# LightwheelAI/street-gaussians-ns

Measured on NVIDIA H100. Metric: rendered frames/sec (fwd+bwd) at 1920x1280, 1M+32x10k Gaussians, higher is better.
Workload: dtype f32

## Files before the change

street-gaussians-ns_b200/csrc/project.cu:

```cuda
#include <stdarg.h>
#include <stdlib.h>
#include <string.h>

#include "sgn_exact.cuh"
#include "sgn_touch.cuh"

static thread_local char g_err[512] = "";
void sgn_set_error(const char* fmt, ...) {
    va_list ap;
    va_start(ap, fmt);
    vsnprintf(g_err, sizeof(g_err), fmt, ap);
    va_end(ap);
}
#include <atomic>
static std::atomic<long long> g_launches{0};
void sgn_count_launch(int n) { g_launches.fetch_add(n, std::memory_order_relaxed); }
extern "C" long long sgn_launch_count(void) { return g_launches.load(std::memory_order_relaxed); }
extern "C" const char* sgn_last_error(void) { return g_err; }
extern "C" int sgn_abi_version(void) { return SGN_ABI_VERSION; }
extern "C" size_t sgn_sizeof_segment(void) { return sizeof(sgn_segment); }
extern "C" size_t sgn_sizeof_segment_grads(void) { return sizeof(sgn_segment_grads); }
extern "C" size_t sgn_sizeof_camera(void) { return sizeof(sgn_camera); }

extern "C" int sgn_upload(const void* host, size_t bytes, void* dev, void* stream) {
    SGN_RANGE("sgn_upload");
    SGN_REQUIRE(host && dev, "sgn_upload: null pointer");
    SGN_CHECK_CUDA(cudaMemcpyAsync(dev, host, bytes, cudaMemcpyHostToDevice, (cudaStream_t)stream));
    return SGN_OK;
}

#define SGN_MAX_SEGMENTS 1024
#define PROJ_THREADS 256
#define CH 128
#define MAX_REST 45
#define MAX_DC (3 * SGN_MAX_FOURIER)

__device__ __forceinline__ sgn_camera sgn_camera_with_view(const sgn_camera& c, const float* __restrict__ view) {
    sgn_camera o = c;
#pragma unroll
    for (int k = 0; k < 12; ++k) o.viewmat[k] = __ldg(view + k);
#pragma unroll
    for (int k = 0; k < 3; ++k) o.cam_pos[k] = __ldg(view + 12 + k);
    return o;
}

__device__ __forceinline__ int find_segment_by_chunk(const int* s_chunk0, int nseg, int c) {
    int lo = 0, hi = nseg - 1;
    while (lo < hi) {
        const int mid = (lo + hi + 1) >> 1;
        if (s_chunk0[mid] <= c) lo = mid; else hi = mid - 1;
    }
    return lo;
}

__device__ __forceinline__ void coop_load(float* __restrict__ dst, const float* __restrict__ src, int n) {
    if ((reinterpret_cast<uintptr_t>(src) & 15u) == 0) {
        const int n4 = n >> 2;
        const float4* s4 = reinterpret_cast<const float4*>(src);
        float4* d4 = reinterpret_cast<float4*>(dst);
        for (int i = threadIdx.x; i < n4; i += blockDim.x) d4[i] = __ldg(s4 + i);
        for (int i = (n4 << 2) + threadIdx.x; i < n; i += blockDim.x) dst[i] = __ldg(src + i);
    } else {
        for (int i = threadIdx.x; i < n; i += blockDim.x) dst[i] = __ldg(src + i);
    }
}
__device__ __forceinline__ void coop_store(float* __restrict__ dst, const float* __restrict__ src, int n) {
    if ((reinterpret_cast<uintptr_t>(dst) & 15u) == 0) {
        const int n4 = n >> 2;
        const float4* s4 = reinterpret_cast<const float4*>(src);
        float4* d4 = reinterpret_cast<float4*>(dst);
        for (int i = threadIdx.x; i < n4; i += blockDim.x) d4[i] = s4[i];
        for (int i = (n4 << 2) + threadIdx.x; i < n; i += blockDim.x) dst[i] = src[i];
    } else {
        for (int i = threadIdx.x; i < n; i += blockDim.x) dst[i] = src[i];
    }
}

template <bool VIEW>
__global__ void __launch_bounds__(CH)
project_fwd_direct_kernel(const sgn_segment* __restrict__ segs, int nseg, const sgn_camera cam_arg,
                   float4* __restrict__ records, int32_t* __restrict__ radii, int32_t* __restrict__ num_tiles_hit,
                   ushort4* __restrict__ tile_bbox, int32_t* __restrict__ tiles_touched, uint32_t* __restrict__ touch_mask,
                   const float* __restrict__ view) {
    sgn_camera cam_view;
    if constexpr (VIEW) cam_view = sgn_camera_with_view(cam_arg, view);
    const sgn_camera& cam = VIEW ? cam_view : cam_arg;
    extern __shared__ int s_chunk0[];
    for (int i = threadIdx.x; i < nseg; i += blockDim.x) s_chunk0[i] = segs[i].chunk0;
    __syncthreads();
    const int si = find_segment_by_chunk(s_chunk0, nseg, blockIdx.x);
    const sgn_segment& sg = segs[si];
    const int i = (blockIdx.x - sg.chunk0) * CH + threadIdx.x;
    const bool active = i < sg.count;
    const size_t g = (size_t)sg.row0 + i;
    const int K = (cam.sh_degree + 1) * (cam.sh_degree + 1);
    bool vis = false;
    ushort4 bb = make_ushort4(0, 0, 0, 0);
    TouchCtx tc = {};
    if (active) {

    float m[3], ls[3], q[4];
#pragma unroll
    for (int k = 0; k < 3; ++k) { m[k] = __ldg(sg.means + 3 * (size_t)i + k); ls[k] = __ldg(sg.scales + 3 * (size_t)i + k); }
    {
        const float4 qq = __ldg(reinterpret_cast<const float4*>(sg.quats) + i);
        q[0] = qq.x; q[1] = qq.y; q[2] = qq.z; q[3] = qq.w;
    }
    const bool filt = cam.filter_3d != nullptr;
    const float sigma = filt ? __ldg(cam.filter_3d[si] + i) : 0.f;
    SgnProj st;
    vis = sgn_project_exact(sg, cam, m, ls, q, st, true, 1.f, cam.antialiased != 0, filt, sigma);

    float rgb[3] = {0.f, 0.f, 0.f};
    float opac = 0.f, comp = 0.f;
    int aux = 0;
    if (vis) {
        float c0[3] = {0.f, 0.f, 0.f};
        for (int f = 0; f < sg.F; ++f) {
            const float w = sg.idft[f];
#pragma unroll
            for (int ch = 0; ch < 3; ++ch) c0[ch] += __ldg(sg.features_dc + ((size_t)i * sg.F + f) * 3 + ch) * w;
        }
        if (cam.sh_degree > 0) {
            float d[3] = {st.mw[0] - cam.cam_pos[0], st.mw[1] - cam.cam_pos[1], st.mw[2] - cam.cam_pos[2]};
            const float n = sqrtf(d[0] * d[0] + d[1] * d[1] + d[2] * d[2]);
            d[0] /= n; d[1] /= n; d[2] /= n;
            float Y[16];
            sgn_sh_basis(cam.sh_degree_to_use, d[0], d[1], d[2], Y);
            const int Kuse = min((cam.sh_degree_to_use + 1) * (cam.sh_degree_to_use + 1), K);
            float acc[3] = {Y[0] * c0[0], Y[0] * c0[1], Y[0] * c0[2]};
            const float* rest = sg.features_rest + (size_t)i * (K - 1) * 3;
            for (int k = 1; k < Kuse; ++k) {
#pragma unroll
                for (int ch = 0; ch < 3; ++ch) acc[ch] += Y[k] * __ldg(rest + (k - 1) * 3 + ch);
            }
#pragma unroll
            for (int ch = 0; ch < 3; ++ch) {
                const float pre = acc[ch] + 0.5f;
                if (pre >= 0.f) aux |= (1 << ch);
                rgb[ch] = pre > 0.f ? pre : 0.f;
            }
        } else {
#pragma unroll
            for (int ch = 0; ch < 3; ++ch) { rgb[ch] = 1.f / (1.f + expf(-c0[ch])); aux |= (1 << ch); }
        }
        opac = 1.f / (1.f + expf(-__ldg(sg.opacities + i)));
        if (filt) opac = opac * st.coef;
        if (cam.antialiased) {
            comp = st.comp;
            opac = opac * comp;
        }
        aux |= SGN_AUX_VISIBLE;
    }
    if (sg.cls == 1) aux |= SGN_AUX_OBJECT;

    float4* rec = records + 3 * g;
    rec[0] = make_float4(st.xy[0], st.xy[1], st.conic[0], st.conic[1]);
    rec[1] = make_float4(st.conic[2], opac, rgb[0], rgb[1]);
    rec[2] = make_float4(rgb[2], vis ? st.pv[2] : 0.f, __int_as_float(aux), comp);
    radii[g] = st.radius;
    num_tiles_hit[g] = vis ? (st.tmax[0] - st.tmin[0]) * (st.tmax[1] - st.tmin[1]) : 0;
    bb = make_ushort4((unsigned short)st.tmin[0], (unsigned short)st.tmin[1],
                      (unsigned short)st.tmax[0], (unsigned short)st.tmax[1]);
    tile_bbox[g] = bb;
    if (vis) tc = make_touch_ctx(make_float4(st.xy[0], st.xy[1], st.conic[0], st.conic[1]), make_float4(st.conic[2], opac, 0.f, 0.f));
    }
    uint32_t mask;
    const int nt = count_touched_tiles(vis, tc, bb, cam.width, cam.height, cam.block_width, mask);
    if (active) {
        tiles_touched[g] = nt;
        touch_mask[g] = mask;
    }
}

__global__ void __launch_bounds__(CH)
project_fwd_staged_kernel(const sgn_segment* __restrict__ segs, int nseg, const sgn_camera cam,
                   float4* __restrict__ records, int32_t* __restrict__ radii, int32_t* __restrict__ num_tiles_hit,
                   ushort4* __restrict__ tile_bbox, int32_t* __restrict__ tiles_touched, uint32_t* __restrict__ touch_mask) {
    extern __shared__ int s_chunk0[];
    __shared__ __align__(16) float s_rest[CH * MAX_REST];
    __shared__ __align__(16) float s_dc[CH * MAX_DC];
    __shared__ __align__(16) float s_means[CH * 3];
    __shared__ __align__(16) float s_scales[CH * 3];
    __shared__ float s_geo[CH][11];
    __shared__ int s_row[CH];
    __shared__ int s_warp_base[CH / 32 + 1];
    for (int i = threadIdx.x; i < nseg; i += blockDim.x) s_chunk0[i] = segs[i].chunk0;
    __syncthreads();
    const int si = find_segment_by_chunk(s_chunk0, nseg, blockIdx.x);
    const sgn_segment& sg = segs[si];
    const int r0 = (blockIdx.x - sg.chunk0) * CH;
    const int rows = min(CH, sg.count - r0);
    const int tid = threadIdx.x, lane = tid & 31, warp = tid >> 5;
    const int K = (cam.sh_degree + 1) * (cam.sh_degree + 1);
    const int nrest = (K - 1) * 3, ndc = sg.F * 3;
    coop_load(s_means, sg.means + 3 * (size_t)r0, rows * 3);
    coop_load(s_scales, sg.scales + 3 * (size_t)r0, rows * 3);
    __syncthreads();

    const bool active = tid < rows;
    const size_t g = (size_t)sg.row0 + r0 + tid;
    const int cls_bit = sg.cls == 1 ? SGN_AUX_OBJECT : 0;
    bool vis = false;
    SgnProj st;
    if (active) {
        const float m[3] = {s_means[3 * tid], s_means[3 * tid + 1], s_means[3 * tid + 2]};
        const float ls[3] = {s_scales[3 * tid], s_scales[3 * tid + 1], s_scales[3 * tid + 2]};
        const float4 qq = __ldg(reinterpret_cast<const float4*>(sg.quats) + r0 + tid);
        const float q[4] = {qq.x, qq.y, qq.z, qq.w};
        const bool filt = cam.filter_3d != nullptr;
        const float sigma = filt ? __ldg(cam.filter_3d[si] + r0 + tid) : 0.f;
        vis = sgn_project_exact(sg, cam, m, ls, q, st, true, 1.f, cam.antialiased != 0, filt, sigma);
        radii[g] = st.radius;
        num_tiles_hit[g] = vis ? (st.tmax[0] - st.tmin[0]) * (st.tmax[1] - st.tmin[1]) : 0;
        tile_bbox[g] = make_ushort4((unsigned short)st.tmin[0], (unsigned short)st.tmin[1],
                                    (unsigned short)st.tmax[0], (unsigned short)st.tmax[1]);
        float4* rec = records + 3 * g;
        rec[0] = make_float4(st.xy[0], st.xy[1], st.conic[0], st.conic[1]);
        if (!vis) {
            rec[1] = make_float4(st.conic[2], 0.f, 0.f, 0.f);
            rec[2] = make_float4(0.f, 0.f, __int_as_float(cls_bit), 0.f);
            tiles_touched[g] = 0;
            touch_mask[g] = 0u;
        }
    }
    const unsigned bal = __ballot_sync(0xffffffffu, vis);
    if (lane == 0) s_warp_base[warp + 1] = __popc(bal);
    __syncthreads();
    if (tid == 0) {
        s_warp_base[0] = 0;
#pragma unroll
        for (int w = 0; w < CH / 32; ++w) s_warp_base[w + 1] += s_warp_base[w];
    }
    __syncthreads();
    const int nvis = s_warp_base[CH / 32];
    if (vis) {
        const int c = s_warp_base[warp] + __popc(bal & ((1u << lane) - 1u));
        s_row[c] = tid;
        float* ge = s_geo[c];
        ge[0] = st.xy[0]; ge[1] = st.xy[1]; ge[2] = st.conic[0]; ge[3] = st.conic[1]; ge[4] = st.conic[2];
        ge[5] = st.pv[2]; ge[6] = st.mw[0]; ge[7] = st.mw[1]; ge[8] = st.mw[2];
        ge[9] = st.comp;
        ge[10] = st.coef;
    }
    __syncthreads();
    if (nvis == 0) return;

    {
        const unsigned inv_rest = nrest > 0 ? (0xffffffffu / (unsigned)nrest) + 1u : 0u;
        const float* __restrict__ rest = sg.features_rest + (size_t)r0 * nrest;
        const int n_rest = nvis * nrest;
        for (int e0 = tid; e0 < n_rest; e0 += 4 * CH) {
            float v[4];
#pragma unroll
            for (int u = 0; u < 4; ++u) {
                const int e = e0 + u * CH;
                if (e < n_rest) {
                    const int r = (int)__umulhi((unsigned)e, inv_rest);
                    v[u] = __ldg(rest + s_row[r] * nrest + (e - r * nrest));
                }
            }
#pragma unroll
            for (int u = 0; u < 4; ++u) {
                const int e = e0 + u * CH;
                if (e < n_rest) s_rest[e] = v[u];
            }
        }
        const unsigned inv_dc = (0xffffffffu / (unsigned)ndc) + 1u;
        const float* __restrict__ dc = sg.features_dc + (size_t)r0 * ndc;
        for (int e = tid; e < nvis * ndc; e += CH) {
            const int r = (int)__umulhi((unsigned)e, inv_dc);
            s_dc[e] = __ldg(dc + s_row[r] * ndc + (e - r * ndc));
        }
    }
    __syncthreads();

    const bool mine = tid < nvis;
    ushort4 bb = make_ushort4(0, 0, 0, 0);
    TouchCtx tc = {};
    size_t gb = 0;
    if (mine) {
        const int row = s_row[tid];
        gb = (size_t)sg.row0 + r0 + row;
        const float* ge = s_geo[tid];
        float c0[3] = {0.f, 0.f, 0.f};
        const float* dcr = s_dc + tid * ndc;
        for (int f = 0; f < sg.F; ++f) {
            const float w = sg.idft[f];
#pragma unroll
            for (int ch = 0; ch < 3; ++ch) c0[ch] += dcr[f * 3 + ch] * w;
        }
        float rgb[3];
        int aux = SGN_AUX_VISIBLE | cls_bit;
        if (cam.sh_degree > 0) {
            float d[3] = {ge[6] - cam.cam_pos[0], ge[7] - cam.cam_pos[1], ge[8] - cam.cam_pos[2]};
            const float n = sqrtf(d[0] * d[0] + d[1] * d[1] + d[2] * d[2]);
            d[0] /= n; d[1] /= n; d[2] /= n;
            float Y[16];
            sgn_sh_basis(cam.sh_degree_to_use, d[0], d[1], d[2], Y);
            const int Kuse = min((cam.sh_degree_to_use + 1) * (cam.sh_degree_to_use + 1), K);
            float acc[3] = {Y[0] * c0[0], Y[0] * c0[1], Y[0] * c0[2]};
            const float* rr = s_rest + tid * nrest;
            for (int k = 1; k < Kuse; ++k) {
#pragma unroll
                for (int ch = 0; ch < 3; ++ch) acc[ch] += Y[k] * rr[(k - 1) * 3 + ch];
            }
#pragma unroll
            for (int ch = 0; ch < 3; ++ch) {
                const float pre = acc[ch] + 0.5f;
                if (pre >= 0.f) aux |= (1 << ch);
                rgb[ch] = pre > 0.f ? pre : 0.f;
            }
        } else {
#pragma unroll
            for (int ch = 0; ch < 3; ++ch) { rgb[ch] = 1.f / (1.f + expf(-c0[ch])); aux |= (1 << ch); }
        }
        float opac = 1.f / (1.f + expf(-__ldg(sg.opacities + r0 + row)));
        if (cam.filter_3d) opac = opac * ge[10];
        if (cam.antialiased) opac = opac * ge[9];
        float4* rec = records + 3 * gb;
        rec[1] = make_float4(ge[4], opac, rgb[0], rgb[1]);
        rec[2] = make_float4(rgb[2], ge[5], __int_as_float(aux), ge[9]);
        bb = tile_bbox[gb];
        tc = make_touch_ctx(make_float4(ge[0], ge[1], ge[2], ge[3]), make_float4(ge[4], opac, 0.f, 0.f));
    }
    if ((warp << 5) >= nvis) return;
    uint32_t mask;
    const int nt = count_touched_tiles(mine, tc, bb, cam.width, cam.height, cam.block_width, mask);
    if (mine) {
        tiles_touched[gb] = nt;
        touch_mask[gb] = mask;
    }
}

static int project_fwd_check(const char* what, const sgn_segment* segs_dev, int nseg, int N, int num_chunks, const sgn_camera* cam,
                             float* records, int32_t* radii, int32_t* num_tiles_hit, uint16_t* tile_bbox,
                             int32_t* tiles_touched, uint32_t* touch_mask) {
    SGN_REQUIRE(segs_dev && cam && records && radii && num_tiles_hit && tile_bbox && tiles_touched && touch_mask,
                "%s: null pointer", what);
    SGN_REQUIRE(nseg >= 1 && nseg <= SGN_MAX_SEGMENTS, "%s: nseg=%d out of range [1,%d]", what, nseg, SGN_MAX_SEGMENTS);
    SGN_REQUIRE(N >= 0 && num_chunks >= 0, "%s: negative size", what);
    SGN_REQUIRE(cam->block_width >= 2 && cam->block_width <= 16, "block_width must be between 2 and 16 (got %d)", cam->block_width);
    SGN_REQUIRE(cam->sh_degree >= 0 && cam->sh_degree <= 3 && cam->sh_degree_to_use >= 0 && cam->sh_degree_to_use <= cam->sh_degree,
                "sh_degree must be in [0,3] and sh_degree_to_use <= sh_degree");
    SGN_REQUIRE((cam->width + cam->block_width - 1) / cam->block_width < 65536 && (cam->height + cam->block_width - 1) / cam->block_width < 65536,
                "image too large for 16-bit tile coordinates");
    SGN_REQUIRE(sgn_aligned16(records), "records must be 16-byte aligned");
    return SGN_OK;
}

extern "C" int sgn_project_fwd_view(const sgn_segment* segs_dev, int nseg, int N, int num_chunks, const sgn_camera* cam,
                                    const float* view, float* records, int32_t* radii, int32_t* num_tiles_hit, uint16_t* tile_bbox,
                                    int32_t* tiles_touched, uint32_t* touch_mask, void* stream) {
    SGN_RANGE("sgn_project_fwd_view");
    if (int rc = project_fwd_check("sgn_project_fwd_view", segs_dev, nseg, N, num_chunks, cam, records, radii, num_tiles_hit, tile_bbox,
                                   tiles_touched, touch_mask)) return rc;
    SGN_REQUIRE(view, "sgn_project_fwd_view: null view");
    if (N == 0 || num_chunks == 0) return SGN_OK;
    project_fwd_direct_kernel<true><<<num_chunks, CH, nseg * sizeof(int), (cudaStream_t)stream>>>(
        segs_dev, nseg, *cam, reinterpret_cast<float4*>(records), radii, num_tiles_hit,
        reinterpret_cast<ushort4*>(tile_bbox), tiles_touched, touch_mask, view);
    SGN_CHECK_LAUNCH("project_fwd_kernel<view>");
    return SGN_OK;
}

extern "C" int sgn_project_fwd(const sgn_segment* segs_dev, int nseg, int N, int num_chunks, const sgn_camera* cam,
                               float* records, int32_t* radii, int32_t* num_tiles_hit, uint16_t* tile_bbox,
                               int32_t* tiles_touched, uint32_t* touch_mask, void* stream) {
    SGN_RANGE("sgn_project_fwd");
    if (int rc = project_fwd_check("sgn_project_fwd", segs_dev, nseg, N, num_chunks, cam, records, radii, num_tiles_hit, tile_bbox,
                                   tiles_touched, touch_mask)) return rc;
    if (N == 0 || num_chunks == 0) return SGN_OK;
    const char* staged_env = getenv("SGN_PROJECT_STAGED");
    if (staged_env && staged_env[0] == '1')
        project_fwd_staged_kernel<<<num_chunks, CH, nseg * sizeof(int), (cudaStream_t)stream>>>(
            segs_dev, nseg, *cam, reinterpret_cast<float4*>(records), radii, num_tiles_hit,
            reinterpret_cast<ushort4*>(tile_bbox), tiles_touched, touch_mask);
    else
        project_fwd_direct_kernel<false><<<num_chunks, CH, nseg * sizeof(int), (cudaStream_t)stream>>>(
            segs_dev, nseg, *cam, reinterpret_cast<float4*>(records), radii, num_tiles_hit,
            reinterpret_cast<ushort4*>(tile_bbox), tiles_touched, touch_mask, nullptr);
    SGN_CHECK_LAUNCH("project_fwd_kernel");
    return SGN_OK;
}

template <bool VIEW = false>
__device__ __forceinline__ void sgn_project_vjp(const sgn_camera& cam, const SgnProj& st, const float v_xy[2], float v_depth,
                                                const float v_conic[3], float vmw[3], float vs[3], float vqr[4],
                                                float* vview = nullptr, bool with_comp = false, float comp = 0.f,
                                                float v_comp = 0.f) {
    const float* W = cam.viewmat;
    const float fx = cam.fx, fy = cam.fy;
    float vpv[3];
    {
        const float rw = 1.f / (st.pv[2] + 1e-6f);
        const float vx = fx * v_xy[0], vy = fy * v_xy[1];
        vpv[0] = vx * rw;
        vpv[1] = vy * rw;
        vpv[2] = -(vx * st.pv[0] + vy * st.pv[1]) * rw * rw + v_depth;
    }
    float vA, vB, vC;
    {
        const float X0 = st.conic[0], X1 = st.conic[1], X2 = st.conic[2];
        const float G0 = v_conic[0], G1 = 0.5f * v_conic[1], G2 = v_conic[2];
        const float a00 = X0 * G0 + X1 * G1, a01 = X0 * G1 + X1 * G2;
        const float a10 = X1 * G0 + X2 * G1, a11 = X1 * G1 + X2 * G2;
        vA = -(a00 * X0 + a01 * X1);
        vB = -(a00 * X1 + a01 * X2) - (a10 * X0 + a11 * X1);
        vC = -(a10 * X1 + a11 * X2);
    }
    if (with_comp) {
        xf T[6], S[6], a, b, c, c00, c11;
#pragma unroll
        for (int k = 0; k < 6; ++k) { T[k] = xf(st.T[k]); S[k] = xf(st.S[k]); }
        sgn_cov2d_blur(T, S, a, b, c, c00, c11);
        sgn_compensation_vjp(c00.v, c11.v, a.v, b.v, c.v, comp, v_comp, vA, vB, vC);
    }
    const float g00 = vA, g01 = 0.5f * vB, g11 = vC;
    const float* T = st.T;
    const float Sf[9] = {st.S[0], st.S[1], st.S[2], st.S[1], st.S[3], st.S[4], st.S[2], st.S[4], st.S[5]};
    float GT[6];
#pragma unroll
    for (int c = 0; c < 3; ++c) {
        GT[c] = g00 * T[c] + g01 * T[3 + c];
        GT[3 + c] = g01 * T[c] + g11 * T[3 + c];
    }
    float vS[9];
#pragma unroll
    for (int r = 0; r < 3; ++r)
#pragma unroll
        for (int c = 0; c < 3; ++c) vS[3 * r + c] = T[r] * GT[c] + T[3 + r] * GT[3 + c];
    float vT[6];
#pragma unroll
    for (int r = 0; r < 2; ++r)
#pragma unroll
        for (int c = 0; c < 3; ++c)
            vT[3 * r + c] = 2.f * (GT[3 * r] * Sf[c] + GT[3 * r + 1] * Sf[3 + c] + GT[3 * r + 2] * Sf[6 + c]);
    const float vJ00 = vT[0] * W[0] + vT[1] * W[1] + vT[2] * W[2];
    const float vJ02 = vT[0] * W[8] + vT[1] * W[9] + vT[2] * W[10];
    const float vJ11 = vT[3] * W[4] + vT[4] * W[5] + vT[5] * W[6];
    const float vJ12 = vT[3] * W[8] + vT[4] * W[9] + vT[5] * W[10];
    {
        const float rz = 1.f / st.pv[2], rz2 = rz * rz, rz3 = rz2 * rz;
        const float vtx = -fx * rz2 * vJ02;
        const float vty = -fy * rz2 * vJ12;
        const float vtz = -fx * rz2 * vJ00 - fy * rz2 * vJ11 + 2.f * fx * st.tx * rz3 * vJ02 + 2.f * fy * st.ty * rz3 * vJ12;
        if (st.clampx == 0) vpv[0] += vtx; else vpv[2] += (st.clampx > 0 ? cam.limx : -cam.limx) * vtx;
        if (st.clampy == 0) vpv[1] += vty; else vpv[2] += (st.clampy > 0 ? cam.limy : -cam.limy) * vty;
        vpv[2] += vtz;
        if constexpr (VIEW) {
            const float J00 = fx * rz, J11 = fy * rz, J02 = -fx * st.tx * rz2, J12 = -fy * st.ty * rz2;
#pragma unroll
            for (int c = 0; c < 3; ++c) {
                vview[c] = vpv[0] * st.mw[c] + J00 * vT[c];
                vview[4 + c] = vpv[1] * st.mw[c] + J11 * vT[3 + c];
                vview[8 + c] = vpv[2] * st.mw[c] + J02 * vT[c] + J12 * vT[3 + c];
            }
#pragma unroll
            for (int r = 0; r < 3; ++r) vview[4 * r + 3] = vpv[r];
        }
    }
#pragma unroll
    for (int c = 0; c < 3; ++c) vmw[c] = W[c] * vpv[0] + W[4 + c] * vpv[1] + W[8 + c] * vpv[2];
    float M[9], vM[9];
#pragma unroll
    for (int r = 0; r < 3; ++r)
#pragma unroll
        for (int c = 0; c < 3; ++c) M[3 * r + c] = st.Rg[3 * r + c] * st.s[c];
#pragma unroll
    for (int r = 0; r < 3; ++r)
#pragma unroll
        for (int c = 0; c < 3; ++c)
            vM[3 * r + c] = 2.f * (vS[3 * r] * M[c] + vS[3 * r + 1] * M[3 + c] + vS[3 * r + 2] * M[6 + c]);
    float vR[9];
#pragma unroll
    for (int c = 0; c < 3; ++c) {
        vs[c] = st.Rg[c] * vM[c] + st.Rg[3 + c] * vM[3 + c] + st.Rg[6 + c] * vM[6 + c];
#pragma unroll
        for (int r = 0; r < 3; ++r) vR[3 * r + c] = vM[3 * r + c] * st.s[c];
    }
    float vqn[4];
    {
        const float w = st.qn[0], x = st.qn[1], y = st.qn[2], z = st.qn[3];
        vqn[0] = 2.f * (x * (vR[7] - vR[5]) + y * (vR[2] - vR[6]) + z * (vR[3] - vR[1]));
        vqn[1] = 2.f * (-2.f * x * (vR[4] + vR[8]) + y * (vR[1] + vR[3]) + z * (vR[2] + vR[6]) + w * (vR[7] - vR[5]));
        vqn[2] = 2.f * (x * (vR[1] + vR[3]) - 2.f * y * (vR[0] + vR[8]) + z * (vR[5] + vR[7]) + w * (vR[2] - vR[6]));
        vqn[3] = 2.f * (x * (vR[2] + vR[6]) + y * (vR[5] + vR[7]) - 2.f * z * (vR[0] + vR[4]) + w * (vR[3] - vR[1]));
    }
    const float dot = vqn[0] * st.qn[0] + vqn[1] * st.qn[1] + vqn[2] * st.qn[2] + vqn[3] * st.qn[3];
#pragma unroll
    for (int k = 0; k < 4; ++k) vqr[k] = (vqn[k] - st.qn[k] * dot) / st.qnorm;
}

template <bool POSE, bool VIEW = false>
__global__ void __launch_bounds__(CH)
project_bwd_kernel(const sgn_segment* __restrict__ segs, const sgn_segment_grads* __restrict__ grads, int nseg,
                   const sgn_camera cam_arg, const float4* __restrict__ records, const int32_t* __restrict__ radii,
                   const float4* __restrict__ v_records, const int chunk_begin, float* __restrict__ pose_partials,
                   const float* __restrict__ view, float* __restrict__ view_partials) {
    sgn_camera cam_view;
    if constexpr (VIEW) cam_view = sgn_camera_with_view(cam_arg, view);
    const sgn_camera& cam = VIEW ? cam_view : cam_arg;
    extern __shared__ int s_chunk0[];
    __shared__ __align__(16) float s_rest[CH * MAX_REST];
    __shared__ __align__(16) float s_dc[CH * MAX_DC];
    __shared__ __align__(16) float s_means[CH * 3];
    __shared__ __align__(16) float s_scales[CH * 3];
    for (int i = threadIdx.x; i < nseg; i += blockDim.x) s_chunk0[i] = segs[i].chunk0;
    __syncthreads();
    const int chunk = chunk_begin + (int)blockIdx.x;
    const int si = find_segment_by_chunk(s_chunk0, nseg, chunk);
    const sgn_segment& sg = segs[si];
    const sgn_segment_grads& gr = grads[si];
    const int r0 = (chunk - sg.chunk0) * CH;
    const int rows = min(CH, sg.count - r0);
    const int K = (cam.sh_degree + 1) * (cam.sh_degree + 1);
    const int nrest = (K - 1) * 3, ndc = sg.F * 3;
    coop_load(s_means, sg.means + 3 * (size_t)r0, rows * 3);
    coop_load(s_scales, sg.scales + 3 * (size_t)r0, rows * 3);
    __syncthreads();
    const int tid = threadIdx.x;
    float gm[3] = {0.f, 0.f, 0.f}, gs[3] = {0.f, 0.f, 0.f}, gq[4] = {0.f, 0.f, 0.f, 0.f};
    float vp[POSE ? SGN_POSE_FLOATS : 1] = {};
    float vv[VIEW ? SGN_VIEW_FLOATS : 1] = {};
    const bool row_vis = (tid < rows) && radii[(size_t)sg.row0 + r0 + tid] > 0;
    if (tid < rows && !row_vis) {
        const int i = r0 + tid;
        gr.opacities[i] = 0.f;
        reinterpret_cast<float4*>(gr.quats)[i] = make_float4(0.f, 0.f, 0.f, 0.f);
        float* grest = s_rest + tid * nrest;
        for (int k = 0; k < nrest; ++k) grest[k] = 0.f;
        float* gdc = s_dc + tid * ndc;
        for (int k = 0; k < ndc; ++k) gdc[k] = 0.f;
    }
    if (row_vis) {
        const int i = r0 + tid;
        const size_t g = (size_t)sg.row0 + i;
        const float4 v0 = v_records[3 * g], v1 = v_records[3 * g + 1], v2 = v_records[3 * g + 2];
        const float v_xy[2] = {v0.x, v0.y};
        const float v_conic[3] = {v0.z, v0.w, v1.x};
        const float v_opac = v1.y;
        const float v_rgb[3] = {v1.z, v1.w, v2.x};
        const float v_depth = v2.y;
        const float4 r1 = records[3 * g + 1], r2 = records[3 * g + 2];
        const int aux = __float_as_int(r2.z);
        const bool filt = cam.filter_3d != nullptr;
        if (!cam.antialiased && !filt) {
            const float o = r1.y;
            gr.opacities[i] = v_opac * o * (1.f - o);
        }
        const float m[3] = {s_means[3 * tid], s_means[3 * tid + 1], s_means[3 * tid + 2]};
        const float ls[3] = {s_scales[3 * tid], s_scales[3 * tid + 1], s_scales[3 * tid + 2]};
        float q[4];
        {
            const float4 qq = __ldg(reinterpret_cast<const float4*>(sg.quats) + i);
            q[0] = qq.x; q[1] = qq.y; q[2] = qq.z; q[3] = qq.w;
        }
        const float sigma = filt ? __ldg(cam.filter_3d[si] + i) : 0.f;
        SgnProj st;
        const bool vis = sgn_project_exact(sg, cam, m, ls, q, st, true, 1.f, false, filt, sigma);
        {
            float vc[3];
            float* grest = s_rest + tid * nrest;
            if (cam.sh_degree > 0) {
                float d[3] = {st.mw[0] - cam.cam_pos[0], st.mw[1] - cam.cam_pos[1], st.mw[2] - cam.cam_pos[2]};
                const float n = sqrtf(d[0] * d[0] + d[1] * d[1] + d[2] * d[2]);
                d[0] /= n; d[1] /= n; d[2] /= n;
                float Y[16];
                sgn_sh_basis(cam.sh_degree_to_use, d[0], d[1], d[2], Y);
                const int Kuse = (cam.sh_degree_to_use + 1) * (cam.sh_degree_to_use + 1);
#pragma unroll
                for (int ch = 0; ch < 3; ++ch) vc[ch] = (aux & (1 << ch)) ? v_rgb[ch] : 0.f;
                for (int k = 1; k < K; ++k) {
                    const float y = (k < Kuse) ? Y[k] : 0.f;
#pragma unroll
                    for (int ch = 0; ch < 3; ++ch) grest[(k - 1) * 3 + ch] = y * vc[ch];
                }
#pragma unroll
                for (int ch = 0; ch < 3; ++ch) vc[ch] *= Y[0];
            } else {
                const float rgb[3] = {r1.z, r1.w, r2.x};
#pragma unroll
                for (int ch = 0; ch < 3; ++ch) vc[ch] = v_rgb[ch] * rgb[ch] * (1.f - rgb[ch]);
                for (int k = 0; k < nrest; ++k) grest[k] = 0.f;
            }
            float* gdc = s_dc + tid * ndc;
            for (int f = 0; f < sg.F; ++f) {
                const float w = sg.idft[f];
#pragma unroll
                for (int ch = 0; ch < 3; ++ch) gdc[f * 3 + ch] = w * vc[ch];
            }
        }
        float v_comp = 0.f, comp = 0.f, v_coef = 0.f;
        if (cam.antialiased || filt) {
            const float s = 1.f / (1.f + expf(-__ldg(sg.opacities + i)));
            float f = 1.f;
            if (cam.antialiased) {
                v_comp = v_opac * s;
                f = r2.w;
                comp = __ldg(reinterpret_cast<const float*>(records) + 12 * g + 11);
            }
            if (filt) {
                v_coef = v_opac * s * f;
                v_comp = v_comp * st.coef;
                f = f * st.coef;
            }
            gr.opacities[i] = v_opac * f * s * (1.f - s);
        }
        if (vis && radii[g] > 0) {
            float vmw[3], vs[3], vqr[4];
            sgn_project_vjp<VIEW>(cam, st, v_xy, v_depth, v_conic, vmw, vs, vqr, vv, cam.antialiased != 0, comp, v_comp);
#pragma unroll
            for (int c = 0; c < 3; ++c) gs[c] = vs[c] * st.s[c];
            if (filt) {
                float r[3];
                sgn_filter_ratios(ls, sigma, r);
                const float vc = v_coef * st.coef;
#pragma unroll
                for (int c = 0; c < 3; ++c) gs[c] = gs[c] * r[c] + vc * (1.f - r[c]);
            }
            if (sg.has_pose) {
                const float* R = sg.R;
#pragma unroll
                for (int c = 0; c < 3; ++c) gm[c] = R[c] * vmw[0] + R[3 + c] * vmw[1] + R[6 + c] * vmw[2];
                const float aw = sg.q[0], ax = sg.q[1], ay = sg.q[2], az = sg.q[3];
                gq[0] = aw * vqr[0] + ax * vqr[1] + ay * vqr[2] + az * vqr[3];
                gq[1] = -ax * vqr[0] + aw * vqr[1] + az * vqr[2] - ay * vqr[3];
                gq[2] = -ay * vqr[0] - az * vqr[1] + aw * vqr[2] + ax * vqr[3];
                gq[3] = -az * vqr[0] + ay * vqr[1] - ax * vqr[2] + aw * vqr[3];
                if constexpr (POSE) {
#pragma unroll
                    for (int r = 0; r < 3; ++r) {
#pragma unroll
                        for (int c = 0; c < 3; ++c) vp[3 * r + c] = vmw[r] * m[c];
                        vp[9 + r] = vmw[r];
                    }
                    vp[12] = vqr[0] * q[0] + vqr[1] * q[1] + vqr[2] * q[2] + vqr[3] * q[3];
                    vp[13] = -vqr[0] * q[1] + vqr[1] * q[0] - vqr[2] * q[3] + vqr[3] * q[2];
                    vp[14] = -vqr[0] * q[2] + vqr[1] * q[3] + vqr[2] * q[0] - vqr[3] * q[1];
                    vp[15] = -vqr[0] * q[3] - vqr[1] * q[2] + vqr[2] * q[1] + vqr[3] * q[0];
                }
            } else {
#pragma unroll
                for (int c = 0; c < 3; ++c) gm[c] = vmw[c];
#pragma unroll
                for (int k = 0; k < 4; ++k) gq[k] = vqr[k];
            }
        }
        reinterpret_cast<float4*>(gr.quats)[i] = make_float4(gq[0], gq[1], gq[2], gq[3]);
    }
    if constexpr (POSE) {
        __shared__ float s_pose[(CH / 32) * SGN_POSE_FLOATS];
        if (sg.has_pose) {
#pragma unroll
            for (int k = 0; k < SGN_POSE_FLOATS; ++k) {
                float x = vp[k];
#pragma unroll
                for (int o = 16; o > 0; o >>= 1) x += __shfl_down_sync(0xffffffffu, x, o);
                if ((tid & 31) == 0) s_pose[(tid >> 5) * SGN_POSE_FLOATS + k] = x;
            }
            __syncthreads();
            if (tid < SGN_POSE_FLOATS) {
                float x = s_pose[tid];
#pragma unroll
                for (int w = 1; w < CH / 32; ++w) x += s_pose[w * SGN_POSE_FLOATS + tid];
                pose_partials[(size_t)chunk * SGN_POSE_FLOATS + tid] = x;
            }
        }
    }
    if constexpr (VIEW) {
        __shared__ float s_view[(CH / 32) * SGN_VIEW_FLOATS];
#pragma unroll
        for (int k = 0; k < SGN_VIEW_FLOATS; ++k) {
            float x = vv[k];
#pragma unroll
            for (int o = 16; o > 0; o >>= 1) x += __shfl_down_sync(0xffffffffu, x, o);
            if ((tid & 31) == 0) s_view[(tid >> 5) * SGN_VIEW_FLOATS + k] = x;
        }
        __syncthreads();
        if (tid < SGN_VIEW_FLOATS) {
            float x = s_view[tid];
#pragma unroll
            for (int w = 1; w < CH / 32; ++w) x += s_view[w * SGN_VIEW_FLOATS + tid];
            view_partials[(size_t)chunk * SGN_VIEW_FLOATS + tid] = x;
        }
    }
// ... 255 lines not shown
```

Before: 438.3.

## Stage SH rest features via per-warp cp.async and coalesce record stores through smem

The projection forward kernel now gathers the SH rest coefficients of visible Gaussians into per-warp shared memory with cp.async. This overlaps the gather with the opacity, DC colour and tile-bbox work, replacing strided per-thread global loads. The 48-byte per-Gaussian records are first written to shared memory and then stored to global memory in a coalesced warp loop. The env-selected staged kernel is removed. The kernel now carries a large static shared-memory buffer, which may lower occupancy.

```diff
diff --git a/street-gaussians-ns_b200/csrc/project.cu b/street-gaussians-ns_b200/csrc/project.cu
--- a/street-gaussians-ns_b200/csrc/project.cu
+++ b/street-gaussians-ns_b200/csrc/project.cu
@@ -76,9 +76,17 @@
     }
 }
 
+__device__ __forceinline__ uint32_t smem_u32(const void* p) { return (uint32_t)__cvta_generic_to_shared(p); }
+__device__ __forceinline__ void cp_async4(void* dst, const void* src) {
+    asm volatile("cp.async.ca.shared.global [%0], [%1], 4;\n" ::"r"(smem_u32(dst)), "l"(src) : "memory");
+}
+__device__ __forceinline__ void cp_async_commit() { asm volatile("cp.async.commit_group;\n" ::: "memory"); }
+template <int N>
+__device__ __forceinline__ void cp_async_wait() { asm volatile("cp.async.wait_group %0;\n" ::"n"(N) : "memory"); }
+
 template <bool VIEW>
 __global__ void __launch_bounds__(CH)
-project_fwd_direct_kernel(const sgn_segment* __restrict__ segs, int nseg, const sgn_camera cam_arg,
+project_fwd_kernel(const sgn_segment* __restrict__ segs, int nseg, const sgn_camera cam_arg,
                    float4* __restrict__ records, int32_t* __restrict__ radii, int32_t* __restrict__ num_tiles_hit,
                    ushort4* __restrict__ tile_bbox, int32_t* __restrict__ tiles_touched, uint32_t* __restrict__ touch_mask,
                    const float* __restrict__ view) {
@@ -86,53 +94,85 @@
     if constexpr (VIEW) cam_view = sgn_camera_with_view(cam_arg, view);
     const sgn_camera& cam = VIEW ? cam_view : cam_arg;
     extern __shared__ int s_chunk0[];
+    __shared__ __align__(16) float s_rest[CH / 32][32 * MAX_REST];
+    __shared__ int s_vrow[CH];
     for (int i = threadIdx.x; i < nseg; i += blockDim.x) s_chunk0[i] = segs[i].chunk0;
     __syncthreads();
     const int si = find_segment_by_chunk(s_chunk0, nseg, blockIdx.x);
     const sgn_segment& sg = segs[si];
-    const int i = (blockIdx.x - sg.chunk0) * CH + threadIdx.x;
+    const int lane = threadIdx.x & 31, warp = threadIdx.x >> 5;
+    const int r0 = (blockIdx.x - sg.chunk0) * CH;
+    const int i = r0 + threadIdx.x;
     const bool active = i < sg.count;
     const size_t g = (size_t)sg.row0 + i;
     const int K = (cam.sh_degree + 1) * (cam.sh_degree + 1);
+    const bool filt = cam.filter_3d != nullptr;
     bool vis = false;
+    SgnProj st;
+    if (active) {
+        float m[3], ls[3], q[4];
+#pragma unroll
+        for (int k = 0; k < 3; ++k) { m[k] = __ldg(sg.means + 3 * (size_t)i + k); ls[k] = __ldg(sg.scales + 3 * (size_t)i + k); }
+#pragma unroll
+        for (int k = 0; k < 4; ++k) q[k] = __ldg(sg.quats + 4 * (size_t)i + k);
+        const float sigma = filt ? __ldg(cam.filter_3d[si] + i) : 0.f;
+        vis = sgn_project_exact(sg, cam, m, ls, q, st, true, 1.f, cam.antialiased != 0, filt, sigma);
+    }
+
+    const unsigned bal = __ballot_sync(0xffffffffu, vis);
+    const int cv = __popc(bal & ((1u << lane) - 1u));
+    const int Kuse = min((cam.sh_degree_to_use + 1) * (cam.sh_degree_to_use + 1), K);
+    const int nrest = (K - 1) * 3, nr = cam.sh_degree > 0 ? (Kuse - 1) * 3 : 0, stride = nr | 1;
+    float* wrest = s_rest[warp];
+    if (vis) s_vrow[(threadIdx.x & ~31) | cv] = lane;
+    __syncwarp();
+    if (nr > 0 && bal) {
+        const float* __restrict__ rest = sg.features_rest + ((size_t)r0 + (warp << 5)) * nrest;
+        const unsigned inv = (0xffffffffu / (unsigned)nr) + 1u;
+        const int n = __popc(bal) * nr;
+        for (int e = lane; e < n; e += 32) {
+            const int v = (int)__umulhi((unsigned)e, inv), k = e - v * nr;
+            cp_async4(wrest + v * stride + k, rest + s_vrow[(threadIdx.x & ~31) | v] * nrest + k);
+        }
+    }
+    cp_async_commit();
+
+    float rgb[3] = {0.f, 0.f, 0.f};
+    float opac = 0.f, comp = 0.f;
+    float c0[3] = {0.f, 0.f, 0.f};
+    int aux = 0;
     ushort4 bb = make_ushort4(0, 0, 0, 0);
     TouchCtx tc = {};
-    if (active) {
-
-    float m[3], ls[3], q[4];
-#pragma unroll
-    for (int k = 0; k < 3; ++k) { m[k] = __ldg(sg.means + 3 * (size_t)i + k); ls[k] = __ldg(sg.scales + 3 * (size_t)i + k); }
-    {
-        const float4 qq = __ldg(reinterpret_cast<const float4*>(sg.quats) + i);
-        q[0] = qq.x; q[1] = qq.y; q[2] = qq.z; q[3] = qq.w;
-    }
-    const bool filt = cam.filter_3d != nullptr;
-    const float sigma = filt ? __ldg(cam.filter_3d[si] + i) : 0.f;
-    SgnProj st;
-    vis = sgn_project_exact(sg, cam, m, ls, q, st, true, 1.f, cam.antialiased != 0, filt, sigma);
-
-    float rgb[3] = {0.f, 0.f, 0.f};
-    float opac = 0.f, comp = 0.f;
-    int aux = 0;
     if (vis) {
-        float c0[3] = {0.f, 0.f, 0.f};
         for (int f = 0; f < sg.F; ++f) {
             const float w = sg.idft[f];
 #pragma unroll
             for (int ch = 0; ch < 3; ++ch) c0[ch] += __ldg(sg.features_dc + ((size_t)i * sg.F + f) * 3 + ch) * w;
         }
+        opac = 1.f / (1.f + expf(-__ldg(sg.opacities + i)));
+        if (filt) opac = opac * st.coef;
+        if (cam.antialiased) {
+            comp = st.comp;
+            opac = opac * comp;
+        }
+        tc = make_touch_ctx(make_float4(st.xy[0], st.xy[1], st.conic[0], st.conic[1]), make_float4(st.conic[2], opac, 0.f, 0.f));
+    }
+    if (active)
+        bb = make_ushort4((unsigned short)st.tmin[0], (unsigned short)st.tmin[1], (unsigned short)st.tmax[0], (unsigned short)st.tmax[1]);
+    cp_async_wait<0>();
+    __syncwarp();
+    if (vis) {
         if (cam.sh_degree > 0) {
             float d[3] = {st.mw[0] - cam.cam_pos[0], st.mw[1] - cam.cam_pos[1], st.mw[2] - cam.cam_pos[2]};
             const float n = sqrtf(d[0] * d[0] + d[1] * d[1] + d[2] * d[2]);
             d[0] /= n; d[1] /= n; d[2] /= n;
             float Y[16];
             sgn_sh_basis(cam.sh_degree_to_use, d[0], d[1], d[2], Y);
-            const int Kuse = min((cam.sh_degree_to_use + 1) * (cam.sh_degree_to_use + 1), K);
             float acc[3] = {Y[0] * c0[0], Y[0] * c0[1], Y[0] * c0[2]};
-            const float* rest = sg.features_rest + (size_t)i * (K - 1) * 3;
+            const float* rr = wrest + cv * stride;
             for (int k = 1; k < Kuse; ++k) {
 #pragma unroll
-                for (int ch = 0; ch < 3; ++ch) acc[ch] += Y[k] * __ldg(rest + (k - 1) * 3 + ch);
+                for (int ch = 0; ch < 3; ++ch) acc[ch] += Y[k] * rr[(k - 1) * 3 + ch];
             }
 #pragma unroll
             for (int ch = 0; ch < 3; ++ch) {
@@ -144,193 +184,27 @@
 #pragma unroll
             for (int ch = 0; ch < 3; ++ch) { rgb[ch] = 1.f / (1.f + expf(-c0[ch])); aux |= (1 << ch); }
         }
-        opac = 1.f / (1.f + expf(-__ldg(sg.opacities + i)));
-        if (filt) opac = opac * st.coef;
-        if (cam.antialiased) {
-            comp = st.comp;
-            opac = opac * comp;
-        }
         aux |= SGN_AUX_VISIBLE;
-    }
-    if (sg.cls == 1) aux |= SGN_AUX_OBJECT;
-
-    float4* rec = records + 3 * g;
-    rec[0] = make_float4(st.xy[0], st.xy[1], st.conic[0], st.conic[1]);
-    rec[1] = make_float4(st.conic[2], opac, rgb[0], rgb[1]);
-    rec[2] = make_float4(rgb[2], vis ? st.pv[2] : 0.f, __int_as_float(aux), comp);
-    radii[g] = st.radius;
-    num_tiles_hit[g] = vis ? (st.tmax[0] - st.tmin[0]) * (st.tmax[1] - st.tmin[1]) : 0;
-    bb = make_ushort4((unsigned short)st.tmin[0], (unsigned short)st.tmin[1],
-                      (unsigned short)st.tmax[0], (unsigned short)st.tmax[1]);
-    tile_bbox[g] = bb;
-    if (vis) tc = make_touch_ctx(make_float4(st.xy[0], st.xy[1], st.conic[0], st.conic[1]), make_float4(st.conic[2], opac, 0.f, 0.f));
     }
     uint32_t mask;
     const int nt = count_touched_tiles(vis, tc, bb, cam.width, cam.height, cam.block_width, mask);
+    if (sg.cls == 1) aux |= SGN_AUX_OBJECT;
+    __syncwarp();
+    float4* wrec = reinterpret_cast<float4*>(wrest);
     if (active) {
+        wrec[3 * lane] = make_float4(st.xy[0], st.xy[1], st.conic[0], st.conic[1]);
+        wrec[3 * lane + 1] = make_float4(st.conic[2], opac, rgb[0], rgb[1]);
+        wrec[3 * lane + 2] = make_float4(rgb[2], vis ? st.pv[2] : 0.f, __int_as_float(aux), comp);
+        radii[g] = st.radius;
+        num_tiles_hit[g] = vis ? (st.tmax[0] - st.tmin[0]) * (st.tmax[1] - st.tmin[1]) : 0;
+        tile_bbox[g] = bb;
         tiles_touched[g] = nt;
         touch_mask[g] = mask;
     }
-}
-
-__global__ void __launch_bounds__(CH)
-project_fwd_staged_kernel(const sgn_segment* __restrict__ segs, int nseg, const sgn_camera cam,
-                   float4* __restrict__ records, int32_t* __restrict__ radii, int32_t* __restrict__ num_tiles_hit,
-                   ushort4* __restrict__ tile_bbox, int32_t* __restrict__ tiles_touched, uint32_t* __restrict__ touch_mask) {
-    extern __shared__ int s_chunk0[];
-    __shared__ __align__(16) float s_rest[CH * MAX_REST];
-    __shared__ __align__(16) float s_dc[CH * MAX_DC];
-    __shared__ __align__(16) float s_means[CH * 3];
-    __shared__ __align__(16) float s_scales[CH * 3];
-    __shared__ float s_geo[CH][11];
-    __shared__ int s_row[CH];
-    __shared__ int s_warp_base[CH / 32 + 1];
-    for (int i = threadIdx.x; i < nseg; i += blockDim.x) s_chunk0[i] = segs[i].chunk0;
-    __syncthreads();
-    const int si = find_segment_by_chunk(s_chunk0, nseg, blockIdx.x);
-    const sgn_segment& sg = segs[si];
-    const int r0 = (blockIdx.x - sg.chunk0) * CH;
-    const int rows = min(CH, sg.count - r0);
-    const int tid = threadIdx.x, lane = tid & 31, warp = tid >> 5;
-    const int K = (cam.sh_degree + 1) * (cam.sh_degree + 1);
-    const int nrest = (K - 1) * 3, ndc = sg.F * 3;
-    coop_load(s_means, sg.means + 3 * (size_t)r0, rows * 3);
-    coop_load(s_scales, sg.scales + 3 * (size_t)r0, rows * 3);
-    __syncthreads();
-
-    const bool active = tid < rows;
-    const size_t g = (size_t)sg.row0 + r0 + tid;
-    const int cls_bit = sg.cls == 1 ? SGN_AUX_OBJECT : 0;
-    bool vis = false;
-    SgnProj st;
-    if (active) {
-        const float m[3] = {s_means[3 * tid], s_means[3 * tid + 1], s_means[3 * tid + 2]};
-        const float ls[3] = {s_scales[3 * tid], s_scales[3 * tid + 1], s_scales[3 * tid + 2]};
-        const float4 qq = __ldg(reinterpret_cast<const float4*>(sg.quats) + r0 + tid);
-        const float q[4] = {qq.x, qq.y, qq.z, qq.w};
-        const bool filt = cam.filter_3d != nullptr;
-        const float sigma = filt ? __ldg(cam.filter_3d[si] + r0 + tid) : 0.f;
-        vis = sgn_project_exact(sg, cam, m, ls, q, st, true, 1.f, cam.antialiased != 0, filt, sigma);
-        radii[g] = st.radius;
-        num_tiles_hit[g] = vis ? (st.tmax[0] - st.tmin[0]) * (st.tmax[1] - st.tmin[1]) : 0;
-        tile_bbox[g] = make_ushort4((unsigned short)st.tmin[0], (unsigned short)st.tmin[1],
-                                    (unsigned short)st.tmax[0], (unsigned short)st.tmax[1]);
-        float4* rec = records + 3 * g;
-        rec[0] = make_float4(st.xy[0], st.xy[1], st.conic[0], st.conic[1]);
-        if (!vis) {
-            rec[1] = make_float4(st.conic[2], 0.f, 0.f, 0.f);
-            rec[2] = make_float4(0.f, 0.f, __int_as_float(cls_bit), 0.f);
-            tiles_touched[g] = 0;
-            touch_mask[g] = 0u;
-        }
-    }
-    const unsigned bal = __ballot_sync(0xffffffffu, vis);
-    if (lane == 0) s_warp_base[warp + 1] = __popc(bal);
-    __syncthreads();
-    if (tid == 0) {
-        s_warp_base[0] = 0;
-#pragma unroll
-        for (int w = 0; w < CH / 32; ++w) s_warp_base[w + 1] += s_warp_base[w];
-    }
-    __syncthreads();
-    const int nvis = s_warp_base[CH / 32];
-    if (vis) {
-        const int c = s_warp_base[warp] + __popc(bal & ((1u << lane) - 1u));
-        s_row[c] = tid;
-        float* ge = s_geo[c];
-        ge[0] = st.xy[0]; ge[1] = st.xy[1]; ge[2] = st.conic[0]; ge[3] = st.conic[1]; ge[4] = st.conic[2];
-        ge[5] = st.pv[2]; ge[6] = st.mw[0]; ge[7] = st.mw[1]; ge[8] = st.mw[2];
-        ge[9] = st.comp;
-        ge[10] = st.coef;
-    }
-    __syncthreads();
-    if (nvis == 0) return;
-
-    {
-        const unsigned inv_rest = nrest > 0 ? (0xffffffffu / (unsigned)nrest) + 1u : 0u;
-        const float* __restrict__ rest = sg.features_rest + (size_t)r0 * nrest;
-        const int n_rest = nvis * nrest;
-        for (int e0 = tid; e0 < n_rest; e0 += 4 * CH) {
-            float v[4];
-#pragma unroll
-            for (int u = 0; u < 4; ++u) {
-                const int e = e0 + u * CH;
-                if (e < n_rest) {
-                    const int r = (int)__umulhi((unsigned)e, inv_rest);
-                    v[u] = __ldg(rest + s_row[r] * nrest + (e - r * nrest));
-                }
-            }
-#pragma unroll
-            for (int u = 0; u < 4; ++u) {
-                const int e = e0 + u * CH;
-                if (e < n_rest) s_rest[e] = v[u];
-            }
-        }
-        const unsigned inv_dc = (0xffffffffu / (unsigned)ndc) + 1u;
-        const float* __restrict__ dc = sg.features_dc + (size_t)r0 * ndc;
-        for (int e = tid; e < nvis * ndc; e += CH) {
-            const int r = (int)__umulhi((unsigned)e, inv_dc);
-            s_dc[e] = __ldg(dc + s_row[r] * ndc + (e - r * ndc));
-        }
-    }
-    __syncthreads();
-
-    const bool mine = tid < nvis;
-    ushort4 bb = make_ushort4(0, 0, 0, 0);
-    TouchCtx tc = {};
-    size_t gb = 0;
-    if (mine) {
-        const int row = s_row[tid];
-        gb = (size_t)sg.row0 + r0 + row;
-        const float* ge = s_geo[tid];
-        float c0[3] = {0.f, 0.f, 0.f};
-        const float* dcr = s_dc + tid * ndc;
-        for (int f = 0; f < sg.F; ++f) {
-            const float w = sg.idft[f];
-#pragma unroll
-            for (int ch = 0; ch < 3; ++ch) c0[ch] += dcr[f * 3 + ch] * w;
-        }
-        float rgb[3];
-        int aux = SGN_AUX_VISIBLE | cls_bit;
-        if (cam.sh_degree > 0) {
-            float d[3] = {ge[6] - cam.cam_pos[0], ge[7] - cam.cam_pos[1], ge[8] - cam.cam_pos[2]};
-            const float n = sqrtf(d[0] * d[0] + d[1] * d[1] + d[2] * d[2]);
-            d[0] /= n; d[1] /= n; d[2] /= n;
-            float Y[16];
-            sgn_sh_basis(cam.sh_degree_to_use, d[0], d[1], d[2], Y);
-            const int Kuse = min((cam.sh_degree_to_use + 1) * (cam.sh_degree_to_use + 1), K);
-            float acc[3] = {Y[0] * c0[0], Y[0] * c0[1], Y[0] * c0[2]};
-            const float* rr = s_rest + tid * nrest;
-            for (int k = 1; k < Kuse; ++k) {
-#pragma unroll
-                for (int ch = 0; ch < 3; ++ch) acc[ch] += Y[k] * rr[(k - 1) * 3 + ch];
-            }
-#pragma unroll
-            for (int ch = 0; ch < 3; ++ch) {
-                const float pre = acc[ch] + 0.5f;
-                if (pre >= 0.f) aux |= (1 << ch);
-                rgb[ch] = pre > 0.f ? pre : 0.f;
-            }
-        } else {
-#pragma unroll
-            for (int ch = 0; ch < 3; ++ch) { rgb[ch] = 1.f / (1.f + expf(-c0[ch])); aux |= (1 << ch); }
-        }
-        float opac = 1.f / (1.f + expf(-__ldg(sg.opacities + r0 + row)));
-        if (cam.filter_3d) opac = opac * ge[10];
-        if (cam.antialiased) opac = opac * ge[9];
-        float4* rec = records + 3 * gb;
-        rec[1] = make_float4(ge[4], opac, rgb[0], rgb[1]);
-        rec[2] = make_float4(rgb[2], ge[5], __int_as_float(aux), ge[9]);
-        bb = tile_bbox[gb];
-        tc = make_touch_ctx(make_float4(ge[0], ge[1], ge[2], ge[3]), make_float4(ge[4], opac, 0.f, 0.f));
-    }
-    if ((warp << 5) >= nvis) return;
-    uint32_t mask;
-    const int nt = count_touched_tiles(mine, tc, bb, cam.width, cam.height, cam.block_width, mask);
-    if (mine) {
-        tiles_touched[gb] = nt;
-        touch_mask[gb] = mask;
-    }
+    __syncwarp();
+    const int wrows = min(32, sg.count - r0 - (warp << 5));
+    float4* dst = records + 3 * ((size_t)sg.row0 + r0 + (warp << 5));
+    for (int k = lane; k < 3 * wrows; k += 32) dst[k] = wrec[k];
 }
 
 static int project_fwd_check(const char* what, const sgn_segment* segs_dev, int nseg, int N, int num_chunks, const sgn_camera* cam,
@@ -349,6 +223,17 @@
     return SGN_OK;
 }
 
+template <bool VIEW>
+static int project_fwd_launch(const sgn_segment* segs_dev, int nseg, int num_chunks, const sgn_camera* cam, const float* view,
+                              float* records, int32_t* radii, int32_t* num_tiles_hit, uint16_t* tile_bbox, int32_t* tiles_touched,
+                              uint32_t* touch_mask, void* stream) {
+    project_fwd_kernel<VIEW><<<num_chunks, CH, nseg * sizeof(int), (cudaStream_t)stream>>>(
+        segs_dev, nseg, *cam, reinterpret_cast<float4*>(records), radii, num_tiles_hit,
+        reinterpret_cast<ushort4*>(tile_bbox), tiles_touched, touch_mask, view);
+    SGN_CHECK_LAUNCH(VIEW ? "project_fwd_kernel<view>" : "project_fwd_kernel");
+    return SGN_OK;
+}
+
 extern "C" int sgn_project_fwd_view(const sgn_segment* segs_dev, int nseg, int N, int num_chunks, const sgn_camera* cam,
                                     const float* view, float* records, int32_t* radii, int32_t* num_tiles_hit, uint16_t* tile_bbox,
                                     int32_t* tiles_touched, uint32_t* touch_mask, void* stream) {
@@ -357,11 +242,8 @@
                                    tiles_touched, touch_mask)) return rc;
     SGN_REQUIRE(view, "sgn_project_fwd_view: null view");
     if (N == 0 || num_chunks == 0) return SGN_OK;
-    project_fwd_direct_kernel<true><<<num_chunks, CH, nseg * sizeof(int), (cudaStream_t)stream>>>(
-        segs_dev, nseg, *cam, reinterpret_cast<float4*>(records), radii, num_tiles_hit,
-        reinterpret_cast<ushort4*>(tile_bbox), tiles_touched, touch_mask, view);
-    SGN_CHECK_LAUNCH("project_fwd_kernel<view>");
-    return SGN_OK;
+    return project_fwd_launch<true>(segs_dev, nseg, num_chunks, cam, view, records, radii, num_tiles_hit, tile_bbox, tiles_touched,
+                                    touch_mask, stream);
 }
 
 extern "C" int sgn_project_fwd(const sgn_segment* segs_dev, int nseg, int N, int num_chunks, const sgn_camera* cam,
@@ -371,17 +253,8 @@
     if (int rc = project_fwd_check("sgn_project_fwd", segs_dev, nseg, N, num_chunks, cam, records, radii, num_tiles_hit, tile_bbox,
                                    tiles_touched, touch_mask)) return rc;
     if (N == 0 || num_chunks == 0) return SGN_OK;
-    const char* staged_env = getenv("SGN_PROJECT_STAGED");
-    if (staged_env && staged_env[0] == '1')
-        project_fwd_staged_kernel<<<num_chunks, CH, nseg * sizeof(int), (cudaStream_t)stream>>>(
-            segs_dev, nseg, *cam, reinterpret_cast<float4*>(records), radii, num_tiles_hit,
-            reinterpret_cast<ushort4*>(tile_bbox), tiles_touched, touch_mask);
-    else
-        project_fwd_direct_kernel<false><<<num_chunks, CH, nseg * sizeof(int), (cudaStream_t)stream>>>(
-            segs_dev, nseg, *cam, reinterpret_cast<float4*>(records), radii, num_tiles_hit,
-            reinterpret_cast<ushort4*>(tile_bbox), tiles_touched, touch_mask, nullptr);
-    SGN_CHECK_LAUNCH("project_fwd_kernel");
-    return SGN_OK;
+    return project_fwd_launch<false>(segs_dev, nseg, num_chunks, cam, nullptr, records, radii, num_tiles_hit, tile_bbox, tiles_touched,
+                                     touch_mask, stream);
 }
 
 template <bool VIEW = false>
```

After: 444.6 (median of 6 runs). +1.4%, better.
